# LorgeN/CART-SLAM

Measured on AMD Instinct MI355X. Metric: stereo-pairs/sec @1242x375xD=128; achieved HBM GB/s vs roofline, higher is better.
Workload: dtype u8

## Files before the change

### cart-slam_amd/cartslam/_lib.py

```python
import ctypes as C
import os

_HERE = os.path.dirname(os.path.abspath(__file__))
LIB_PATH = os.environ.get("CART_ENGINE_LIB") or os.path.join(os.path.dirname(_HERE), "build", "libcart_engine.so")


class EngineParams(C.Structure):
    _fields_ = [(n, C.c_int) for n in (
        "device_id", "width", "height", "min_disparity", "num_disparities", "paths", "p1", "p2",
        "uniqueness_ratio", "smoothing_radius", "smoothing_iterations", "max_inflight")]


class PlaneParams(C.Structure):
    _fields_ = [(n, C.c_int) for n in (
        "horizontal_min", "horizontal_max", "vertical_min", "vertical_max",
        "horizontal_center", "vertical_center")]

    def as_tuple(self):
        return tuple(getattr(self, n) for n, _ in self._fields_)


class LaunchPlan(C.Structure):
    _fields_ = [("frames_per_launch", C.c_int), ("plan", C.c_int), ("slabs_written", C.c_int)]


PLAN_AUTO, PLAN_SLABS, PLAN_FUSED_UP, PLAN_BAND_UP = -1, 0, 1, 2
OPT_PLAN, OPT_PLAN_MIN_FRAMES, OPT_CHUNK_FRAMES = 0, 1, 2
OPT_BAND_ROWS, OPT_BAND_PROBE = 6, 7
OPT_FLOW_GATHER = 8
OPT_SPEC_S8_ZERO_INVALID, OPT_SPEC_S7_REPLICATE_BORDER, OPT_SPEC_S5_TOP2 = 3, 4, 5


class FlowParams(C.Structure):
    _fields_ = [(n, C.c_int) for n in ("levels", "radius", "refine_radius", "block", "median")]


FLOW_MAX_LEVELS = 6


class PlacementReport(C.Structure):
    _fields_ = [("ms_first", C.c_float), ("ms_kept", C.c_float), ("ms_fastest_seen", C.c_float), ("ms_slowest_seen", C.c_float),
                ("seconds", C.c_float), ("units", C.c_int), ("candidates", C.c_int), ("mode", C.c_int), ("stop_reason", C.c_int)]


PRED_PLANEFIT, PRED_PLANECLUSTER = 0, 1
PLANEFIT_MAX_PLANES = 100
PLANEFIT_THRESHOLD = 0.01


ORB_DEFAULT_FEATURES, ORB_MAX_FEATURES, ORB_LEVELS, ORB_DESCRIPTOR_BYTES = 5000, 65536, 8, 32

# ... 356 lines not shown
```

### cart-slam_amd/cartslam/engine.py

```python
import collections
import ctypes as C

import numpy as np

from . import _lib
from ._lib import DenseEgoParams, ModelTrackColorParams, ModelTrackParams, EgoCamera, EgoParams, EngineParams, FusionParams, LocalBAParams, MatchParams, MotionParams, ObjectParams, PlaceParams, PlaneMapParams, PlaneParams, PoseGraphParams, SuperpixelParams, VoxelMapParams

INVALID = -32768


class EngineError(RuntimeError):
    pass


def _stream_ptr():
    import torch
    return C.c_void_p(torch.cuda.current_stream().cuda_stream)


def _geom(t, inner):
    if not t.is_cuda:
        raise EngineError("tensor must live on the GPU")
    batched = t.dim() == inner + 2
    if t.dim() not in (inner + 1, inner + 2):
# ... 82 lines not shown
    def __del__(self):
        try:
            self.close()
        except Exception:
            pass

    def _check(self, rc, what):
        if rc != 0:
            raise EngineError(f"{what}: " + self._lib.cart_last_error(self._h).decode())

    def set_plan(self, plan, min_frames=1):
        code = {"auto": _lib.PLAN_AUTO, "slabs": _lib.PLAN_SLABS, "fused_up": _lib.PLAN_FUSED_UP, "band_up": _lib.PLAN_BAND_UP}[plan]
        self._check(self._lib.cart_engine_set_option(self._h, _lib.OPT_PLAN, code), "cart_engine_set_option")
        self._check(self._lib.cart_engine_set_option(self._h, _lib.OPT_PLAN_MIN_FRAMES, int(min_frames)), "cart_engine_set_option")

    def set_spec_variants(self, s8_zero_invalid=False, s7_replicate_border=False, s5_top2=False):
        self._check(self._lib.cart_engine_set_option(self._h, _lib.OPT_SPEC_S5_TOP2, 1 if s5_top2 else 0), "cart_engine_set_option")
        self._check(self._lib.cart_engine_set_option(self._h, _lib.OPT_SPEC_S8_ZERO_INVALID, 1 if s8_zero_invalid else 0), "cart_engine_set_option")
        self._check(self._lib.cart_engine_set_option(self._h, _lib.OPT_SPEC_S7_REPLICATE_BORDER, 1 if s7_replicate_border else 0), "cart_engine_set_option")

    def set_band_rows(self, k, probe=False):
        self._check(self._lib.cart_engine_set_option(self._h, _lib.OPT_BAND_ROWS, int(k)), "cart_engine_set_option")
        self._check(self._lib.cart_engine_set_option(self._h, _lib.OPT_BAND_PROBE, 1 if probe else 0), "cart_engine_set_option")

    def set_chunk_frames(self, n):
        self._check(self._lib.cart_engine_set_option(self._h, _lib.OPT_CHUNK_FRAMES, int(n)), "cart_engine_set_option")

    def describe_plan(self, n_frames):
        lp = _lib.LaunchPlan()
        self._check(self._lib.cart_engine_describe_plan(self._h, int(n_frames), C.byref(lp)), "cart_engine_describe_plan")
        return {"frames_per_launch": lp.frames_per_launch, "plan": {0: "slabs", 1: "fused_up", 2: "band_up"}[lp.plan],
                "slabs_written": lp.slabs_written}

    def copy_narrow(self, dst, src, workgroups=0):
        nbytes = src.numel() * src.element_size()
        if dst.numel() * dst.element_size() != nbytes or not dst.is_contiguous() or not src.is_contiguous():
            raise EngineError("copy_narrow needs two contiguous tensors of the same byte size")
        if not (dst.is_cuda or dst.is_pinned()) or not (src.is_cuda or src.is_pinned()):
            raise EngineError("copy_narrow needs device tensors or pinned host tensors")
        self._check(self._lib.cart_copy_narrow(self._h, C.c_void_p(dst.data_ptr()), C.c_void_p(src.data_ptr()), nbytes, int(workgroups),
                                               _stream_ptr()), "cart_copy_narrow")
        return dst

    def tune_placement(self, n_frames, max_tries=8, max_extra_bytes=0, report=False):
        r = _lib.PlacementReport()
        cap = C.c_size_t(-1).value if max_extra_bytes is None else int(max_extra_bytes)
# ... 1512 lines not shown
```

### cart-slam_amd/csrc/cart_engine.hip

```cpp
#include <chrono>
#include <cstdio>

#include "engine_host.h"

using namespace cart_amd;

namespace cart_amd {

thread_local std::string g_last_error;
thread_local int g_last_slot = 0;

int fail(const std::string &msg) {
    g_last_error = msg;
    return -1;
}

int SlotLease::begin(cart_engine *e, int n, hipStream_t stream) {
    if (n <= 0 || n > (int)e->slots.size()) return fail("n_frames must be in [1, max_inflight]");
    std::unique_lock<std::mutex> lk(e->mu);
    int s0 = -1;
    for (;;) {
        const int total = (int)e->slots.size();
        int oldest = -1;
        unsigned long long oldest_seq = ~0ull;
// ... 79 lines not shown
    int blk = 0, nd = 0;
    const int lpb = agg_lines_per_block(g.D);
    for (int i = 0; i < g.P; ++i) {
        if (!((mask >> i) & 1u)) continue;
        DirDesc &d = a.dirs[nd++];
        d.dx = order8[i].dx; d.dy = order8[i].dy; d.path = order8[i].path;
        if (d.dy == 0) { d.nlines = g.h; d.jmin = 0; }
        else if (d.dx == 0) { d.nlines = g.w; d.jmin = 0; }
        else { d.nlines = g.w + g.h - 1; d.jmin = d.dx > 0 ? -(g.h - 1) : 0; }
        d.blk0 = blk;
        blk += (d.nlines + lpb - 1) / lpb;
    }
    a.ndirs = nd;
    a.blocks_per_frame = blk;
    a.cen_l = e->cen_l; a.cen_r = e->cen_r; a.slabs = SlabTable{};
}

struct Options {
    int plan, plan_min_frames, chunk_frames;
    bool timing;
    int spec;
    int band_rows;
    bool band_probe;
};
Options snapshot_options(const cart_engine *e) {
    return Options{e->opt_plan, e->opt_plan_min_frames, e->chunk_frames, e->timing, e->opt_spec, e->opt_band_rows, e->opt_band_probe != 0};
}

int plan_for(const cart_engine *e, const Options &o, int n) {
    if (o.spec & 4) return CART_PLAN_SLABS;
    const bool band_ok = wta_band_supported(e->g, o.band_rows, o.band_probe);
    if (o.plan == CART_PLAN_AUTO) {
        if (band_ok && !o.band_probe && n >= e->auto_band_min_frames) return CART_PLAN_BAND_UP;
        return n >= e->auto_fused_min_frames ? CART_PLAN_FUSED_UP : CART_PLAN_SLABS;
    }
    if (n < o.plan_min_frames) return CART_PLAN_SLABS;
    if (o.plan == CART_PLAN_BAND_UP && !band_ok) return CART_PLAN_SLABS;
    return o.plan;
}

int validate(const cart_engine_params *p) {
    if (!p) return fail("params is NULL");
    if (p->width < 16 || p->height < 8 || p->width > 16384 || p->height > 16384) return fail("unsupported image size");
    const bool post_only = p->num_disparities == 0 && p->paths == 0;
    if (!post_only && !(p->num_disparities == 64 || p->num_disparities == 128 || p->num_disparities == 256))
        return fail("num_disparities must be 64, 128 or 256");
    if (!post_only && !(p->paths == 4 || p->paths == 8)) return fail("paths must be 4 or 8");
    if (p->min_disparity < 0 || p->min_disparity > 64) return fail("min_disparity must be in [0, 64]");
    if (p->p1 < 0 || p->p2 < p->p1 || p->p2 + 31 > 255) return fail("need 0 <= p1 <= p2 and 31 + p2 <= 255");
// ... 54 lines not shown
    SlabTable t{};
    if (s0 < 0 || n < 1 || n > kMaxLaunchFrames || s0 + n > sp.slots || sp.group_slots < 1) return t;
    for (int f = 0; f < n; ++f) {
        const int s = s0 + f, gi = s / sp.group_slots;
        uint8_t *b = subst && (*subst)[gi] ? (*subst)[gi] : sp.base[gi];
        t.frame[f] = b + (size_t)(s % sp.group_slots) * sp.slot_bytes;
    }
    return t;
}

template <typename F>
void launch_agg_wta(cart_engine *e, const Options &opt, const SlabTable &slabs, size_t s0, int n, hipStream_t st, F between) {
    const Geometry &g = e->g;
    uint32_t *cl = e->cen_l + s0 * g.census_elems, *cr = e->cen_r + s0 * g.census_elems;
    uint16_t *wl = e->wta_l + s0 * g.npx;
    uint32_t *rpk = e->right_pk + s0 * g.npx;
    const int plan = plan_for(e, opt, n);
    const bool fused = plan == CART_PLAN_FUSED_UP && e->rv_partial, band = plan == CART_PLAN_BAND_UP;
    AggArgs a = fused ? e->agg_fused : e->agg;
    a.cen_l = cl; a.cen_r = cr; a.slabs = slabs;
    a.ckpt_rows = band && !opt.band_probe ? opt.band_rows : 0;
    launch_aggregate(a, n, st);
    between();
    if (band) launch_wta_band(cl, cr, slabs, wl, rpk, g, e->uniq_thr, n, opt.band_rows, opt.band_probe, st);
    else if (fused) launch_wta_fused(cl, cr, slabs, wl, rpk, e->rv_partial + s0 * wta_fused_partial_elems(g), g, e->uniq_thr, n, st);
    else launch_wta(slabs, wl, rpk, g, e->uniq_thr, n, st, (opt.spec & 4) != 0);
}

}

extern "C" {

void cart_engine_default_params(cart_engine_params *p) {
    if (!p) return;
    std::memset(p, 0, sizeof(*p));
    p->device_id = 0;
    p->min_disparity = 4;
    p->num_disparities = 256;
    p->paths = 4;
    p->p1 = 10; p->p2 = 120;
    p->uniqueness_ratio = 12;
    p->smoothing_radius = -1;
    p->smoothing_iterations = 5;
    p->max_inflight = 12;
}

int cart_engine_create(const cart_engine_params *params, cart_engine **out) {
// ... 88 lines not shown
    if (!e) return fail("engine is NULL");
    std::lock_guard<std::mutex> lk(e->mu);
    switch (option) {
        case CART_OPT_PLAN:
            if (value < CART_PLAN_AUTO || value > CART_PLAN_BAND_UP) return fail("unknown plan");
            e->opt_plan = value;
            return 0;
        case CART_OPT_PLAN_MIN_FRAMES:
            if (value < 1) return fail("min frames must be >= 1");
            e->opt_plan_min_frames = value;
            return 0;
        case CART_OPT_CHUNK_FRAMES:
            if (value < 1 || value > kMaxLaunchFrames) return fail("chunk frames must be in [1, 64]");
            e->chunk_frames = value;
            return 0;
        case CART_OPT_BAND_ROWS:
            if (value != 1 && value != 4 && value != 8 && value != 16) return fail("band rows must be 4, 8 or 16 (1 with the probe)");
            e->opt_band_rows = value;
            return 0;
        case CART_OPT_BAND_PROBE:
            if (value != 0 && value != 1) return fail("the band probe is 0 or 1");
            e->opt_band_probe = value;
            return 0;
        case CART_OPT_FLOW_GATHER:
            if (value != 0 && value != 1) return fail("the flow gather option is 0 or 1");
            e->opt_flow_gather = value;
            return 0;
        case CART_OPT_SPEC_S8_ZERO_INVALID:
        case CART_OPT_SPEC_S7_REPLICATE_BORDER:
        case CART_OPT_SPEC_S5_TOP2: {
            if (value != 0 && value != 1) return fail("spec variants are 0 or 1");
            const int bit = option == CART_OPT_SPEC_S8_ZERO_INVALID ? 1 : option == CART_OPT_SPEC_S7_REPLICATE_BORDER ? 2 : 4;
            e->opt_spec = value ? (e->opt_spec | bit) : (e->opt_spec & ~bit);
            return 0;
        }
        default: return fail("unknown option");
    }
}

int cart_engine_get_option(cart_engine *e, int option, int *value) {
    if (!e || !value) return fail("bad arguments");
    std::lock_guard<std::mutex> lk(e->mu);
    switch (option) {
        case CART_OPT_PLAN: *value = e->opt_plan; return 0;
        case CART_OPT_PLAN_MIN_FRAMES: *value = e->opt_plan_min_frames; return 0;
        case CART_OPT_CHUNK_FRAMES: *value = e->chunk_frames; return 0;
        case CART_OPT_BAND_ROWS: *value = e->opt_band_rows; return 0;
        case CART_OPT_BAND_PROBE: *value = e->opt_band_probe; return 0;
        case CART_OPT_FLOW_GATHER: *value = e->opt_flow_gather; return 0;
        case CART_OPT_SPEC_S8_ZERO_INVALID: *value = (e->opt_spec & 1) ? 1 : 0; return 0;
        case CART_OPT_SPEC_S7_REPLICATE_BORDER: *value = (e->opt_spec & 2) ? 1 : 0; return 0;
        case CART_OPT_SPEC_S5_TOP2: *value = (e->opt_spec & 4) ? 1 : 0; return 0;
        default: return fail("unknown option");
    }
}

int cart_engine_describe_plan(cart_engine *e, int n_frames, cart_launch_plan *out) {
    if (!e || !out) return fail("bad arguments");
    if (e->post_only) return fail("this engine was created without SGM workspaces (num_disparities = 0)");
    if (n_frames < 1) return fail("n_frames must be positive");
    std::lock_guard<std::mutex> lk(e->mu);
    const Options o = snapshot_options(e);
    out->frames_per_launch = std::min(n_frames, o.chunk_frames);
    out->plan = plan_for(e, o, out->frames_per_launch);
    out->slabs_written = out->plan == CART_PLAN_FUSED_UP || (out->plan == CART_PLAN_BAND_UP && !o.band_probe) ? e->g.P - 1 : e->g.P;
    return 0;
}

namespace {
float probe_placement(cart_engine *e, const Options &opt, const SlabTable &slabs, size_t s0, int n, hipEvent_t ev0, hipEvent_t ev1) {
    const Geometry &g = e->g;
// ... 394 lines not shown
```

### cart-slam_amd/csrc/engine_host.h

```cpp
#pragma once

#include <algorithm>
#include <cmath>
#include <condition_variable>
#include <cstring>
#include <mutex>
#include <new>
#include <string>
#include <vector>

#include "engine_internal.h"

#pragma GCC visibility push(hidden)

namespace cart_amd {

extern thread_local std::string g_last_error;
extern thread_local int g_last_slot;

int fail(const std::string &msg);

int check_positive(const char *name, double v);
int check_camera(const cart_ego_camera *cam);
int check_pose(const char *name, const double *m);
// ... 13 lines not shown
};
int check_pitched(const Extent &x);
bool overlap(const Extent &a, const Extent &b);
int check_outputs_apart(const Extent *all, int first_output, int n);

#define HIP_TRY(expr)                                                                               \
    do {                                                                                            \
        hipError_t _e = (expr);                                                                     \
        if (_e != hipSuccess)                                                                       \
            return fail(std::string(#expr) + ": " + hipGetErrorString(_e) + " (" + __FILE__ + ":" + \
                        std::to_string(__LINE__) + ")");                                           \
    } while (0)

struct Slot {
    bool busy = false;
    hipEvent_t done = nullptr;
    int owner = -1;
    hipStream_t last_stream = nullptr;
    bool used = false;
    unsigned long long released_seq = 0;
};

constexpr int kBandRowsDefault = 8;
constexpr int kBandAutoMinFrames = 4;
constexpr int kMaxTimings = 8;
constexpr int kTimingRing = 256;

struct TimingRec {
    hipEvent_t ev[kMaxTimings + 1] = {};
    const char *names[kMaxTimings] = {};
    int n = 0;
};

struct SlabPool {
    std::vector<uint8_t *> base;
    int group_slots = 0;
    int slots = 0;
    size_t slot_bytes = 0;
    int groups() const { return (int)base.size(); }
    int slots_of(int gi) const { return std::min(group_slots, slots - gi * group_slots); }
    size_t bytes_of(int gi) const { return (size_t)slots_of(gi) * slot_bytes; }
    uint8_t *slot_ptr(int s) const { return base[s / group_slots] + (size_t)(s % group_slots) * slot_bytes; }
};

}

// ... 3 lines not shown
    float uniq;
    uint16_t *uniq_thr = nullptr;
    uint8_t *gray_l = nullptr, *gray_r = nullptr;
    uint32_t *cen_l = nullptr, *cen_r = nullptr;
    uint32_t *cen_l_alloc = nullptr, *cen_r_alloc = nullptr;
    size_t cen_slack = 0;
    uint16_t *wta_l = nullptr;
    uint32_t *right_pk = nullptr;
    int16_t *tmp_a = nullptr, *tmp_b = nullptr;
    int32_t *ccl_work = nullptr;
    uint32_t *rv_partial = nullptr;
    uint8_t *flow_ws = nullptr;
    uint8_t *flow_pyr_ws = nullptr;
    int32_t *ccl_stats_ws = nullptr;
    unsigned *sp_votes = nullptr;
    std::vector<void *> bufs;
    cart_amd::AggArgs agg;
    cart_amd::AggArgs agg_fused;
    cart_amd::SlabPool slab_pool;
    int auto_fused_min_frames = 1 << 30;
    int opt_plan = CART_PLAN_AUTO;
    int auto_band_min_frames = 1 << 30;
    int opt_band_rows = cart_amd::kBandRowsDefault, opt_band_probe = 0;
    int opt_plan_min_frames = 1;
    int opt_flow_gather = 0;
    int opt_spec = 0;
    std::mutex mu;
    std::condition_variable cv;
    std::vector<cart_amd::Slot> slots;
    unsigned long long release_counter = 0;
    int chunk_frames = cart_amd::kLaunchFrames;
    bool post_only = false;
    bool timing = false;
    int timing_every = 1;
    unsigned long long timing_calls = 0;
    std::vector<cart_amd::TimingRec> ring;
    size_t ring_calls = 0;
};

namespace cart_amd {

class SlotLease {
   public:
    SlotLease() = default;
    SlotLease(const SlotLease &) = delete;
    SlotLease &operator=(const SlotLease &) = delete;
// ... 83 lines not shown
```

### cart-slam_amd/csrc/engine_internal.h

```cpp
#pragma once

#include <hip/hip_runtime.h>
#include <stddef.h>
#include <stdint.h>

#include "cart_engine.h"

namespace cart_amd {

constexpr int kMaxPaths = 8;
constexpr int kWtaTileX = 64;
constexpr int kMaxBatchArgs = 128;
constexpr uint32_t kWtaInvalid = 0xFFFFu;
constexpr int kSlabChunkOrder[16] = {0, 8, 1, 9, 2, 10, 3, 11, 4, 12, 5, 13, 6, 14, 7, 15};

struct Geometry {
    int w, h, D, P;
    int min_disp, p1, p2;
    int cpitch;
    int cpadl;
    size_t npx;
    size_t census_elems;
    size_t slab_bytes;
};
// ... 34 lines not shown
    ImageBatch b{}; b.ptr = ptr; b.step = step; b.frame_stride = frame_stride; return b;
}

struct OutBatch {
    int16_t *ptr;
    size_t step, frame_stride;
    int16_t *frames[kLaunchFrames];
    int scattered;
};
inline OutBatch strided_out(int16_t *ptr, size_t step, size_t frame_stride) {
    OutBatch b{}; b.ptr = ptr; b.step = step; b.frame_stride = frame_stride; return b;
}

void launch_census(const ImageBatch &left, const ImageBatch &right, int channels, int n_frames,
                   uint8_t *gray_l, uint8_t *gray_r, uint32_t *cen_l, uint32_t *cen_r, uint32_t *right_pk,
                   const Geometry &g, hipStream_t s);
int agg_lines_per_block(int D);
int agg_residency_cap(int ndirs, int D, int n_frames, bool hsplit = false);
bool agg_hsplit(const Geometry &g, int ndirs, int n_frames);
void launch_aggregate(const AggArgs &a, int n_frames, hipStream_t s);
void launch_wta(const SlabTable &slabs, uint16_t *wta_l, uint32_t *right_pk, const Geometry &g, const uint16_t *thr,
                int n_frames, hipStream_t s, bool top2 = false);
constexpr int kUpPath = 1;
size_t wta_fused_partial_elems(const Geometry &g);
void launch_wta_fused(const uint32_t *cen_l, const uint32_t *cen_r, const SlabTable &slabs, uint16_t *wta_l, uint32_t *right_pk,
                      uint32_t *partial, const Geometry &g, const uint16_t *thr, int n_frames, hipStream_t s);
bool wta_band_supported(const Geometry &g, int K, bool probe);
void launch_wta_band(const uint32_t *cen_l, const uint32_t *cen_r, const SlabTable &slabs, uint16_t *wta_l, uint32_t *right_pk,
                     const Geometry &g, const uint16_t *thr, int n_frames, int K, bool probe, hipStream_t s);
void launch_uniq_table(float u, uint16_t *out_dev, hipStream_t s);
void uniq_table_host(float u, uint16_t *out);
void launch_post(const uint16_t *wta_l, const uint32_t *right_pk, const uint8_t *gray_l, const OutBatch &out, const Geometry &g, int n_frames, hipStream_t s,
                 int spec = 0);
bool post_interp_fusable(int radius, int min_disp16, int max_disp);
void launch_post_interp(const uint16_t *wta_l, const uint32_t *right_pk, const uint8_t *gray_l, const OutBatch &out, const Geometry &g, int n_frames,
                        hipStream_t s, int spec, int min_disp16, int max_disp);

void launch_interpolate(const int16_t *src, size_t src_step, size_t src_fs, const OutBatch &dst, int w, int h, int radius,
                        int min_disp16, int max_disp, int n_frames, hipStream_t s);
void launch_dir_derivative(const int16_t *disp, size_t step, size_t fs, int16_t *out, size_t ostep, size_t ofs,
                           int32_t *hist512, int w, int h, int n_frames, hipStream_t s);
struct FrameTable { const void *p[kLaunchFrames]; int scattered; };
void launch_plane_derivative(const int16_t *disp, size_t step, size_t fs, int16_t *out, size_t ostep, size_t ofs,
                             int32_t *hist256, size_t hist_fs, int w, int h, int n_frames, hipStream_t s,
                             const FrameTable *disp_table = nullptr, const FrameTable *out_table = nullptr);
struct ClassifyParams { cart_plane_params p[kMaxBatchArgs]; };
void launch_classify(const int16_t *deriv, size_t step, size_t fs, const ClassifyParams &params, int per_frame,
                     uint8_t *planes, size_t pstep, size_t pfs, int w, int h, int n_frames, hipStream_t s,
                     const FrameTable *deriv_table = nullptr, const FrameTable *planes_table = nullptr);
void launch_ccl(const uint8_t *planes, size_t pstep, size_t pfs, int32_t *work, int32_t *ids, size_t istep, size_t ifs,
                int32_t *ncomp, int w, int h, int n_frames, hipStream_t s, int32_t *stat = nullptr, int32_t *seg = nullptr,
                cart_component *table = nullptr, int max_components = 0);
// ... 598 lines not shown
```

### cart-slam_amd/csrc/sgm_aggregate.hip

```cpp
#include <algorithm>

#include "sgm_device.h"

namespace cart_amd {


typedef uint32_t u32x4_g4 __attribute__((ext_vector_type(4), aligned(4)));
__device__ __forceinline__ void ld_u32x16(const uint32_t *ubase, unsigned &byte_off, uint32_t (&r)[16]) {
    const CART_GLOBAL char *b = (const CART_GLOBAL char *)sgpr(ubase) + pin_v(byte_off);
#pragma unroll
    for (int i = 0; i < 4; ++i) {
        const u32x4_g4 v = *(const CART_GLOBAL u32x4_g4 *)(b + 16 * i);
        r[4 * i + 0] = v.x; r[4 * i + 1] = v.y; r[4 * i + 2] = v.z; r[4 * i + 3] = v.w;
    }
}

__device__ __forceinline__ void load_census(const uint32_t *pl, unsigned &off_l, const uint32_t *pr, unsigned &off_r, CensusRegs &c) {
    c.fl = ld_u32(pl, off_l);
    ld_u32x16(pr, off_r, c.r);
}

constexpr int HS_PF = 8;
template <int LPP, int DX>
__device__ __forceinline__ void hscan_sliding(uint32_t (&st)[8], uint32_t &mm, const uint32_t *&pl, unsigned &lo_l, const uint32_t *&pr,
// ... 9 lines not shown
    }
    auto group = [&]() {
#pragma unroll
        for (int j = 0; j < 16; ++j) {
            constexpr int M = 15;
            const int slot = j % HS_PF;
#pragma unroll
            for (int k = 0; k < 16; ++k) xr[k] = ffl[slot] ^ win[(DX > 0 ? k + j : k - j + 16) & M];
            win[(DX > 0 ? j : 15 - j) & M] = fnw[slot];
            __builtin_amdgcn_sched_barrier(0);
            ffl[slot] = ld_u32(pl + (j + HS_PF) * DX, lo_l);
            fnw[slot] = ld_u32(pr + (j + HS_PF + 1) * DX, lo_n);
            __builtin_amdgcn_sched_barrier(0);
            agg_step<LPP>(st, mm, xr, sel_lo, sel_hi, p1p1, p2p2, sgpr(po + j * ostride) + pin_v(lo_o));
            __builtin_amdgcn_sched_barrier(0);
        }
        pl += 16 * DX; pr += 16 * DX; po += 16 * ostride;
    };
    group();
    for (int gi = 1; gi < groups; ++gi) group();
}

constexpr int kHsCostDwords = 2 * 2 * 64 * 4;

template <int LPP>
__device__ __forceinline__ v4u agg_step_c(uint32_t (&a)[8], uint32_t &mm, const uint32_t (&c)[8], uint32_t sel_lo, uint32_t sel_hi,
                                          uint32_t p1p1, uint32_t p2p2) {
    const uint32_t mp2 = mm + p2p2;
    const uint32_t lo0 = perm(a[7], dpp_mov<DPP_ROW_SHR1>(a[7]), sel_lo);
    const uint32_t hi7 = perm(dpp_mov<DPP_ROW_SHL1>(a[0]), a[0], sel_hi);
    uint32_t n[8];
#pragma unroll
    for (int i = 0; i < 8; ++i) {
        const uint32_t lo = i == 0 ? lo0 : a[i - 1];
        const uint32_t hi = i == 7 ? hi7 : a[i + 1];
        uint32_t t = pk_min(lo, hi) + p1p1;
        t = pk_min3(t, a[i], mp2);
        n[i] = (t - mm) + c[i];
    }
    const v4u q = {perm(n[1], n[0], 0x06040200u), perm(n[3], n[2], 0x06040200u), perm(n[5], n[4], 0x06040200u), perm(n[7], n[6], 0x06040200u)};
    uint32_t x = pk_min(pk_min3(n[0], n[1], n[2]), pk_min3(n[3], n[4], pk_min3(n[5], n[6], n[7])));
    x = pk_min(x, __builtin_amdgcn_alignbit(x, x, 16));
    mm = group_allmin<LPP>(x);
#pragma unroll
    for (int i = 0; i < 8; ++i) a[i] = n[i];
    return q;
}

template <int LPP, int DX>
__device__ __forceinline__ void hsplit_producer(const uint32_t *pl, unsigned lo_l, const uint32_t *pr, unsigned lo_r, int w, uint32_t *cost, int lane) {
    auto emit = [&](int parity, const uint32_t (&c)[8]) {
        v4u *dst = reinterpret_cast<v4u *>(cost) + parity * 128 + lane;
        dst[0] = v4u{c[0], c[1], c[2], c[3]};
        dst[64] = v4u{c[4], c[5], c[6], c[7]};
        lds_barrier();
    };
    const int groups = w / 16;
    if (groups > 0) {
        uint32_t win[16], ffl[HS_PF], fnw[HS_PF];
        ld_u32x16(pr, lo_r, win);
        unsigned lo_n = lo_r + (DX > 0 ? 15u * 4u : 0u);
#pragma unroll
        for (int q = 0; q < HS_PF; ++q) {
            ffl[q] = ld_u32(pl + q * DX, lo_l);
            fnw[q] = ld_u32(pr + (q + 1) * DX, lo_n);
        }
        auto group = [&]() {
#pragma unroll
            for (int j = 0; j < 16; ++j) {
                const int slot = j % HS_PF;
// ... 346 lines not shown
```

### cart-slam_amd/csrc/sgm_device.h

```cpp
#pragma once

#include <type_traits>

#include "engine_internal.h"

namespace cart_amd {

typedef uint16_t u16x2 __attribute__((ext_vector_type(2)));
typedef uint32_t v4u __attribute__((ext_vector_type(4)));

__device__ __forceinline__ uint32_t pk_min(uint32_t a, uint32_t b) {
    return __builtin_bit_cast(uint32_t, __builtin_elementwise_min(__builtin_bit_cast(u16x2, a), __builtin_bit_cast(u16x2, b)));
}
__device__ __forceinline__ uint32_t pk_min3(uint32_t a, uint32_t b, uint32_t c) {
#if defined(__gfx950__)
    uint32_t r;
    asm("v_pk_minimum3_f16 %0, %1, %2, %3" : "=v"(r) : "v"(a), "v"(b), "v"(c));
    return r;
#else
    return pk_min(pk_min(a, b), c);
#endif
}
__device__ __forceinline__ void keep_f16_denormals() { __builtin_amdgcn_s_setreg(1 | (6 << 6) | (1 << 11), 3); }
__device__ __forceinline__ uint32_t pk_add(uint32_t a, uint32_t b) {
// ... 84 lines not shown
        uint32_t t = pk_min(lo, hi) + p1p1;
        t = pk_min3(t, a[i], mp2);
        uint32_t u = t - mm;
        asm volatile("" : "+v"(u));
        uint32_t lo_sum = (uint32_t)__builtin_popcount(xr[15 - i]) + u;
        asm volatile("" : "+v"(lo_sum));
        n[i] = ((uint32_t)__builtin_popcount(xr[7 - i]) << 16) + lo_sum;
    }
    if constexpr (STORE) {
        uint4 o;
        o.x = perm(n[1], n[0], 0x06040200u); o.y = perm(n[3], n[2], 0x06040200u);
        o.z = perm(n[5], n[4], 0x06040200u); o.w = perm(n[7], n[6], 0x06040200u);
        const v4u q = {o.x, o.y, o.z, o.w};
        if (store_row) __builtin_nontemporal_store(q, (CART_GLOBAL v4u *)po);
    } else {
        (void)po; (void)store_row;
    }
    mm = path_min<LPP>(n);
#pragma unroll
    for (int i = 0; i < 8; ++i) a[i] = n[i];
}

template <int LPP>
struct Win {
    static constexpr int P = 64 / LPP;
    static constexpr int D = 16 * LPP;
    static constexpr int RL = 16 + P - 1;
    static constexpr int RS = LPP == 4 ? 40 : LPP == 8 ? 36 : 34;
    static constexpr int NE = LPP * RL;
    static constexpr int NLD = (NE + 63) / 64;
    static constexpr int BUF = LPP * RS;
    static_assert(RS >= RL && RS % 32 == (P / 2) % 32, "region stride");
};

template <int LPP>
struct WinLane {
    unsigned goff[Win<LPP>::NLD];
    int lslot[Win<LPP>::NLD];
    int rbase;
    __device__ __forceinline__ void init(int lane) {
        using WN = Win<LPP>;
#pragma unroll
        for (int i = 0; i < WN::NLD; ++i) {
            const int e = min(64 * i + lane, WN::NE - 1);
            const int g = e / WN::RL, o = e - g * WN::RL;
            goff[i] = (unsigned)(WN::D - 16 - 16 * g + o) * 4u;
// ... 29 lines not shown
```

### cart-slam_amd/csrc/sgm_wta.hip

```cpp
#include <cstdlib>
#include <type_traits>

#include "sgm_device.h"

namespace cart_amd {

__host__ __device__ constexpr int rv_slot(int i) { return i + (i >> 4); }
__host__ __device__ constexpr int rv_size(int n) { return ((n + (n >> 4) + 1) + 3) & ~3; }
__host__ __device__ constexpr int rv_row_slots(int cols, int D, bool padded) { return ((padded ? rv_size(cols + D - 1) : cols + D) + 7) & ~7; }
__host__ __device__ constexpr uint32_t rv_key16(uint32_t key32, int cols) {
    return ((((key32 >> 16) << (cols == 32 ? 5 : 4)) | (key32 & (uint32_t)(cols - 1))) & 0xffffu);
}
__host__ __device__ constexpr uint32_t rv_key32(uint32_t key16, int e, int cols, int D) {
    const int sh = cols == 32 ? 5 : 4, base = D - 1 - e;
    return ((key16 >> sh) << 16) | (uint32_t)(base + (((int)(key16 & (uint32_t)(cols - 1)) - base) & (cols - 1)));
}

__device__ __forceinline__ uint32_t pk_sub_sat(uint32_t a, uint32_t b) {
    return __builtin_bit_cast(uint32_t, __builtin_elementwise_sub_sat(__builtin_bit_cast(u16x2, a), __builtin_bit_cast(u16x2, b)));
}

__host__ __device__ __forceinline__ uint32_t uniq_threshold(uint32_t bc, float u) {
    if (bc == 0) return 0;
    if (!(u > 0.f)) return 4095u;
// ... 136 lines not shown
        p1p1 = (uint32_t)g.p1 * 0x10001u; p2p2 = (uint32_t)g.p2 * 0x10001u;
        sel_lo = gl == 0 ? 0x05040d0du : 0x05040302u;
        sel_hi = gl == LPP - 1 ? 0x0d0d0302u : 0x05040302u;
        wl.init(lane);
        const ptrdiff_t cen0 = (ptrdiff_t)frame * (ptrdiff_t)g.census_elems + g.cpadl + xw0;
        pw0 = cen_r + uniform(cen0 - g.min_disp - (D - 1));
        pl0 = cen_l + uniform(cen0);
        lo_l = (unsigned)pg * 4u;
        const int xbase = min(xw0, g.w - 1), xc = min(x, g.w - 1);
        ps0 = slabs + uniform((ptrdiff_t)xbase * D);
        lo_s = (unsigned)((xc - xbase) * D + d0);
        cpitch = g.cpitch; row_bytes = (ptrdiff_t)g.w * D; slab_bytes = (ptrdiff_t)g.slab_bytes;
    }
    __device__ __forceinline__ void load_census_row(int y, uint32_t (&win)[WN::NLD], uint32_t &fl) {
        const uint32_t *pw = pw0 + (ptrdiff_t)y * cpitch;
#pragma unroll
        for (int i = 0; i < WN::NLD; ++i) win[i] = ld_u32(pw, wl.goff[i]);
        fl = ld_u32(pl0 + (ptrdiff_t)y * cpitch, lo_l);
    }
    __device__ __forceinline__ v4u load_slab(int y, int path) {
        const uint8_t *ps = ps0 + (ptrdiff_t)y * row_bytes + (ptrdiff_t)path * slab_bytes;
        return __builtin_nontemporal_load((const CART_GLOBAL v4u *)((const CART_GLOBAL char *)sgpr(ps) + pin_v(lo_s)));
    }
    template <bool SKIP_UP, int NS>
    __device__ __forceinline__ void load_slab_row(int y, uint32_t (&sv)[NS][4]) {
#pragma unroll
        for (int p = 0; p < (SKIP_UP ? NS + 1 : NS); ++p) {
            if (SKIP_UP && p == kUpPath) continue;
            const int k = SKIP_UP && p > kUpPath ? p - 1 : p;
            const v4u v = load_slab(y, p);
            sv[k][0] = v.x; sv[k][1] = v.y; sv[k][2] = v.z; sv[k][3] = v.w;
        }
    }
};

template <int LPP, bool TOP2 = false>
__global__ __launch_bounds__(256) void wta_kernel(WtaArgs a) {
    extern __shared__ __attribute__((aligned(16))) uint16_t s_lds[];
    constexpr int D = LPP * 16;
    constexpr int DP = D + 8;
    constexpr int PPP = 256 / LPP;
    constexpr int NPASS = kWtaTileX / PPP;
    uint16_t *wta_l = a.wta_l;
    uint32_t *right_pk = a.right_pk;
    const Geometry &g = a.g;
    const int x0 = blockIdx.x * kWtaTileX, y = blockIdx.y, frame = blockIdx.z;
    const uint8_t *slabs = a.slabs.frame[frame];
    const int grp = threadIdx.x / LPP, gl = threadIdx.x % LPP, d0 = gl * 16;
    __shared__ uint32_t s_rv[kWtaTileX + D];
    for (int i = threadIdx.x; i < kWtaTileX + D; i += 256) s_rv[i] = 0xffffffffu;
    __syncthreads();

// ... 85 lines not shown
}

void launch_wta(const SlabTable &slabs, uint16_t *wta_l, uint32_t *right_pk, const Geometry &g, const uint16_t *thr,
                int n_frames, hipStream_t s, bool top2) {
    dim3 grid((g.w + kWtaTileX - 1) / kWtaTileX, g.h, n_frames), block(256);
    const size_t lds = (size_t)kWtaTileX * (g.D + 8) * sizeof(uint16_t);
    WtaArgs a{slabs, wta_l, right_pk, g, thr, g.P, {0, 1, 2, 3, 4, 5, 6, 7}};
    with_lpp(g.D, [&](auto lpp) {
        constexpr int LPP = decltype(lpp)::value;
        if (top2) hipLaunchKernelGGL((wta_kernel<LPP, true>), grid, block, lds, s, a);
        else hipLaunchKernelGGL((wta_kernel<LPP>), grid, block, lds, s, a);
    });
}

struct BandArgs {
    const uint32_t *cen_l, *cen_r;
    SlabTable slabs;
    uint16_t *wta_l;
    uint32_t *right_pk;
    Geometry g;
    const uint16_t *thr;
};

template <int LPP, int K, bool RECOMP = true>
__global__ __launch_bounds__(64 * LPP, 4) void wta_band_kernel(BandArgs a) {
    using WN = Win<LPP>;
    constexpr int D = WN::D, P = WN::P, NT = 64 * LPP, NP = kMaxPaths, NS = RECOMP ? NP - 1 : NP;
    constexpr int DP = D + 8;
    constexpr int NRV = kWtaTileX + D;
    static_assert(P * LPP == 64 && NT / LPP == kWtaTileX, "one pixel of the tile per lane group");
    __shared__ __attribute__((aligned(16))) uint16_t s_sum[kWtaTileX * DP];
    __shared__ uint32_t s_rv[2][NRV];
    __shared__ uint32_t s_win[RECOMP ? LPP : 1][WN::BUF];
    __shared__ uint16_t s_thr[2048];
    const Geometry &g = a.g;
    keep_f16_denormals();
    const int x0 = blockIdx.x * kWtaTileX, frame = blockIdx.z;
    const int y0 = (int)blockIdx.y * K, y1 = min(g.h, y0 + K);

    for (int i = threadIdx.x; i < 2 * NRV; i += NT) (&s_rv[0][0])[i] = 0xffffffffu;
    for (int i = threadIdx.x; i < 2048; i += NT) s_thr[i] = a.thr[i];

    UpSweep<LPP> sw;
    sw.init(g, a.cen_l, a.cen_r, a.slabs.frame[frame], frame, x0);
    const int gl = sw.gl, d0 = sw.d0, xl = sw.xl, x = sw.x;
    const bool valid = sw.valid;
    uint32_t *wbuf = &s_win[RECOMP ? sw.wid : 0][0];
    uint32_t cw[WN::NLD], cfl, sv[NS][4];

    uint32_t st[8], mm = 0;
#pragma unroll
    for (int i = 0; i < 8; ++i) st[i] = 0;
    if constexpr (RECOMP) sw.load_census_row(y1 - 1, cw, cfl);
    if (RECOMP && y1 < g.h) {
        const v4u v = sw.load_slab(y1, kUpPath);
#pragma unroll
        for (int q = 0; q < 4; ++q) {
            st[2 * q] = perm(0u, v[q], 0x0c010c00u);
            st[2 * q + 1] = perm(0u, v[q], 0x0c030c02u);
        }
        mm = path_min<LPP>(st);
    }
    sw.template load_slab_row<RECOMP>(y1 - 1, sv);
    lds_barrier();

    auto row = [&](int y, auto last_c) {
        constexpr bool LAST = decltype(last_c)::value;
        uint32_t *rvb = &s_rv[y & 1][0];
        uint32_t sm[8];
        if constexpr (RECOMP) {
#pragma unroll
            for (int i = 0; i < WN::NLD; ++i) wbuf[sw.wl.lslot[i]] = cw[i];
            CensusRegs c;
            c.fl = cfl;
            win_read<LPP>(wbuf, sw.wl.rbase, c.r);
            uint32_t xr[16];
            agg_xor(c, xr);
            if constexpr (!LAST) sw.load_census_row(y - 1, cw, cfl);
            agg_step<LPP, false>(st, mm, xr, sw.sel_lo, sw.sel_hi, sw.p1p1, sw.p2p2, nullptr);
            sum_from_state(sm, st);
        } else {
#pragma unroll
            for (int k = 0; k < 8; ++k) sm[k] = 0;
        }
#pragma unroll
        for (int k = 0; k < NS; ++k) sum_add_slab(sm, sv[k]);
        if constexpr (!LAST) sw.template load_slab_row<RECOMP>(y - 1, sv);
        v4u *dst = reinterpret_cast<v4u *>(s_sum + xl * DP + d0);
        dst[0] = v4u{sm[0], sm[1], sm[2], sm[3]};
        dst[1] = v4u{sm[4], sm[5], sm[6], sm[7]};
        if (valid) rv_scatter(rvb + (xl + D - 1 - d0), sm, d0);
        uint32_t pk, T, tot;
        wta_best_and_sum<LPP>(sm, d0, s_thr, pk, T, tot);
        if (gl == 0 && valid) {
            const WtaPick w = wta_decide<D>(pk, T, tot, s_sum + xl * DP);
            a.wta_l[(size_t)frame * g.npx + (size_t)y * g.w + x] = (uint16_t)wta_subpixel<D>(w);
        }
        lds_barrier();
        for (int pi = threadIdx.x; pi < kWtaTileX + D - 1; pi += NT) {
            const int p = x0 - (D - 1) + pi;
            const uint32_t best = rvb[pi];
            rvb[pi] = 0xffffffffu;
            if (p >= 0 && p < g.w && best != 0xffffffffu) atomicMin(&a.right_pk[(size_t)frame * g.npx + (size_t)y * g.w + p], best);
        }
    };
    for (int y = y1 - 1; y > y0; --y) row(y, std::false_type{});
    row(y0, std::true_type{});
}

bool wta_band_supported(const Geometry &g, int K, bool probe) { return g.D == 128 && g.P == kMaxPaths && (K == 4 || K == 8 || K == 16 || (probe && K == 1)); }

void launch_wta_band(const uint32_t *cen_l, const uint32_t *cen_r, const SlabTable &slabs, uint16_t *wta_l, uint32_t *right_pk,
                     const Geometry &g, const uint16_t *thr, int n_frames, int K, bool probe, hipStream_t s) {
    dim3 grid((g.w + kWtaTileX - 1) / kWtaTileX, (g.h + K - 1) / K, n_frames), block(64 * (g.D / 16));
    BandArgs a{cen_l, cen_r, slabs, wta_l, right_pk, g, thr};
    if (probe) {
        switch (K) {
            case 1: hipLaunchKernelGGL((wta_band_kernel<8, 1, false>), grid, block, 0, s, a); break;
            case 4: hipLaunchKernelGGL((wta_band_kernel<8, 4, false>), grid, block, 0, s, a); break;
            case 8: hipLaunchKernelGGL((wta_band_kernel<8, 8, false>), grid, block, 0, s, a); break;
            default: hipLaunchKernelGGL((wta_band_kernel<8, 16, false>), grid, block, 0, s, a); break;
        }
        return;
    }
    switch (K) {
        case 4: hipLaunchKernelGGL((wta_band_kernel<8, 4>), grid, block, 0, s, a); break;
        case 8: hipLaunchKernelGGL((wta_band_kernel<8, 8>), grid, block, 0, s, a); break;
        default: hipLaunchKernelGGL((wta_band_kernel<8, 16>), grid, block, 0, s, a); break;
    }
}

constexpr int fused_waves(int lpp) { return lpp >= 16 ? 4 : 2; }
constexpr int kFusedRB = 16;
inline int fused_waves_for(const Geometry &g) { return g.D >= 256 && g.w >= 1600 ? 2 * fused_waves(16) : fused_waves(g.D / 16); }


struct FusedArgs {
    const uint32_t *cen_l, *cen_r;
    SlabTable slabs;
    uint16_t *wta_l;
    uint32_t *partial;
    Geometry g;
    const uint16_t *thr;
    int xcd_frames;
// ... 263 lines not shown
```

### include/cart_engine.h

```cpp
#ifndef CART_ENGINE_H
#define CART_ENGINE_H

#include <stddef.h>
#include <stdint.h>

#ifdef __cplusplus
extern "C" {
#endif

#define CART_DISPARITY_INVALID (-32768)

enum { CART_PLANE_HORIZONTAL = 0, CART_PLANE_VERTICAL = 1, CART_PLANE_UNKNOWN = 2 };

typedef struct cart_engine cart_engine;

typedef struct {
    int device_id;
    int width, height;
    int min_disparity;
    int num_disparities;
    int paths;
    int p1, p2;
    int uniqueness_ratio;
    int smoothing_radius;
// ... 2 lines not shown
} cart_engine_params;

typedef struct {
    int horizontal_min, horizontal_max;
    int vertical_min, vertical_max;
    int horizontal_center, vertical_center;
} cart_plane_params;

void cart_engine_default_params(cart_engine_params *p);

int cart_engine_create(const cart_engine_params *params, cart_engine **out);
void cart_engine_destroy(cart_engine *engine);

enum { CART_PLAN_AUTO = -1, CART_PLAN_SLABS = 0, CART_PLAN_FUSED_UP = 1, CART_PLAN_BAND_UP = 2 };
enum {
    CART_OPT_PLAN = 0,
    CART_OPT_PLAN_MIN_FRAMES = 1,
    CART_OPT_CHUNK_FRAMES = 2,
    CART_OPT_SPEC_S8_ZERO_INVALID = 3,
    CART_OPT_SPEC_S7_REPLICATE_BORDER = 4,
    CART_OPT_SPEC_S5_TOP2 = 5,
    CART_OPT_BAND_ROWS = 6,
    CART_OPT_BAND_PROBE = 7,
    CART_OPT_FLOW_GATHER = 8
};
int cart_engine_set_option(cart_engine *engine, int option, int value);
int cart_engine_get_option(cart_engine *engine, int option, int *value);
typedef struct {
    int frames_per_launch;
    int plan;
    int slabs_written;
} cart_launch_plan;
int cart_engine_describe_plan(cart_engine *engine, int n_frames, cart_launch_plan *out);

enum { CART_PLACE_MODE_UNKNOWN = 0, CART_PLACE_MODE_FAST = 1, CART_PLACE_MODE_MIXED = 2, CART_PLACE_MODE_UNIFORM = 3 };
enum { CART_PLACE_STOP_NOTHING_TO_DO = 0, CART_PLACE_STOP_FAST_FOUND = 1, CART_PLACE_STOP_UNIFORM = 2, CART_PLACE_STOP_TRIES = 3,
       CART_PLACE_STOP_TIME = 4, CART_PLACE_STOP_MEMORY = 5 };
typedef struct {
    float ms_first, ms_kept;
    float ms_fastest_seen, ms_slowest_seen;
    float seconds;
    int units, candidates;
    int mode, stop_reason;
} cart_placement_report;
int cart_engine_tune_placement(cart_engine *engine, int n_frames, int max_tries, size_t max_extra_bytes, cart_placement_report *report);

const char *cart_last_error(const cart_engine *engine);
// ... 600 lines not shown
```

Measured before the change: 5965.

## Recompute the up-right diagonal path inside the band WTA kernel

The band WTA kernel can now recompute the up-right diagonal aggregation path in registers, alongside the already recomputed vertical up path, instead of loading that path's cost slab for every row. Neighbouring lanes exchange their diagonal state each row through a double-buffered shared-memory array, and the tile's left-edge column is read from the slab. The row is seeded from the slab at the band's bottom boundary. The aim is to cut the per-row HBM slab reads in the WTA pass, at the cost of more ALU work, extra LDS traffic and higher register pressure. A new option, on by default, selects the diagonal variant whenever the band plan runs.

```diff
diff --git a/cart-slam_amd/cartslam/_lib.py b/cart-slam_amd/cartslam/_lib.py
--- a/cart-slam_amd/cartslam/_lib.py
+++ b/cart-slam_amd/cartslam/_lib.py
@@ -27,6 +27,7 @@
 PLAN_AUTO, PLAN_SLABS, PLAN_FUSED_UP, PLAN_BAND_UP = -1, 0, 1, 2
 OPT_PLAN, OPT_PLAN_MIN_FRAMES, OPT_CHUNK_FRAMES = 0, 1, 2
 OPT_BAND_ROWS, OPT_BAND_PROBE = 6, 7
+OPT_BAND_DIAG = 9
 OPT_FLOW_GATHER = 8
 OPT_SPEC_S8_ZERO_INVALID, OPT_SPEC_S7_REPLICATE_BORDER, OPT_SPEC_S5_TOP2 = 3, 4, 5
 
diff --git a/cart-slam_amd/cartslam/engine.py b/cart-slam_amd/cartslam/engine.py
--- a/cart-slam_amd/cartslam/engine.py
+++ b/cart-slam_amd/cartslam/engine.py
@@ -128,6 +128,14 @@
     def set_band_rows(self, k, probe=False):
         self._check(self._lib.cart_engine_set_option(self._h, _lib.OPT_BAND_ROWS, int(k)), "cart_engine_set_option")
         self._check(self._lib.cart_engine_set_option(self._h, _lib.OPT_BAND_PROBE, 1 if probe else 0), "cart_engine_set_option")
+
+    def set_band_diag(self, on=True):
+        self._check(self._lib.cart_engine_set_option(self._h, _lib.OPT_BAND_DIAG, 1 if on else 0), "cart_engine_set_option")
+
+    def get_option(self, option):
+        v = C.c_int(0)
+        self._check(self._lib.cart_engine_get_option(self._h, int(option), C.byref(v)), "cart_engine_get_option")
+        return int(v.value)
 
     def set_chunk_frames(self, n):
         self._check(self._lib.cart_engine_set_option(self._h, _lib.OPT_CHUNK_FRAMES, int(n)), "cart_engine_set_option")
diff --git a/cart-slam_amd/csrc/cart_engine.hip b/cart-slam_amd/csrc/cart_engine.hip
--- a/cart-slam_amd/csrc/cart_engine.hip
+++ b/cart-slam_amd/csrc/cart_engine.hip
@@ -125,9 +125,10 @@
     int spec;
     int band_rows;
     bool band_probe;
+    bool band_diag;
 };
 Options snapshot_options(const cart_engine *e) {
-    return Options{e->opt_plan, e->opt_plan_min_frames, e->chunk_frames, e->timing, e->opt_spec, e->opt_band_rows, e->opt_band_probe != 0};
+    return Options{e->opt_plan, e->opt_plan_min_frames, e->chunk_frames, e->timing, e->opt_spec, e->opt_band_rows, e->opt_band_probe != 0, e->opt_band_diag != 0};
 }
 
 int plan_for(const cart_engine *e, const Options &o, int n) {
@@ -228,7 +229,7 @@
     a.ckpt_rows = band && !opt.band_probe ? opt.band_rows : 0;
     launch_aggregate(a, n, st);
     between();
-    if (band) launch_wta_band(cl, cr, slabs, wl, rpk, g, e->uniq_thr, n, opt.band_rows, opt.band_probe, st);
+    if (band) launch_wta_band(cl, cr, slabs, wl, rpk, g, e->uniq_thr, n, opt.band_rows, opt.band_probe, opt.band_diag, st);
     else if (fused) launch_wta_fused(cl, cr, slabs, wl, rpk, e->rv_partial + s0 * wta_fused_partial_elems(g), g, e->uniq_thr, n, st);
     else launch_wta(slabs, wl, rpk, g, e->uniq_thr, n, st, (opt.spec & 4) != 0);
 }
@@ -363,6 +364,10 @@
             if (value != 0 && value != 1) return fail("the band probe is 0 or 1");
             e->opt_band_probe = value;
             return 0;
+        case CART_OPT_BAND_DIAG:
+            if (value != 0 && value != 1) return fail("the band diagonal option is 0 or 1");
+            e->opt_band_diag = value;
+            return 0;
         case CART_OPT_FLOW_GATHER:
             if (value != 0 && value != 1) return fail("the flow gather option is 0 or 1");
             e->opt_flow_gather = value;
@@ -388,6 +393,7 @@
         case CART_OPT_CHUNK_FRAMES: *value = e->chunk_frames; return 0;
         case CART_OPT_BAND_ROWS: *value = e->opt_band_rows; return 0;
         case CART_OPT_BAND_PROBE: *value = e->opt_band_probe; return 0;
+        case CART_OPT_BAND_DIAG: *value = e->opt_band_diag; return 0;
         case CART_OPT_FLOW_GATHER: *value = e->opt_flow_gather; return 0;
         case CART_OPT_SPEC_S8_ZERO_INVALID: *value = (e->opt_spec & 1) ? 1 : 0; return 0;
         case CART_OPT_SPEC_S7_REPLICATE_BORDER: *value = (e->opt_spec & 2) ? 1 : 0; return 0;
diff --git a/cart-slam_amd/csrc/engine_host.h b/cart-slam_amd/csrc/engine_host.h
--- a/cart-slam_amd/csrc/engine_host.h
+++ b/cart-slam_amd/csrc/engine_host.h
@@ -59,6 +59,7 @@
 };
 
 constexpr int kBandRowsDefault = 8;
+constexpr int kBandDiagDefault = 1;
 constexpr int kBandAutoMinFrames = 4;
 constexpr int kMaxTimings = 8;
 constexpr int kTimingRing = 256;
@@ -108,6 +109,7 @@
     int opt_plan = CART_PLAN_AUTO;
     int auto_band_min_frames = 1 << 30;
     int opt_band_rows = cart_amd::kBandRowsDefault, opt_band_probe = 0;
+    int opt_band_diag = cart_amd::kBandDiagDefault;
     int opt_plan_min_frames = 1;
     int opt_flow_gather = 0;
     int opt_spec = 0;
diff --git a/cart-slam_amd/csrc/engine_internal.h b/cart-slam_amd/csrc/engine_internal.h
--- a/cart-slam_amd/csrc/engine_internal.h
+++ b/cart-slam_amd/csrc/engine_internal.h
@@ -80,12 +80,13 @@
 void launch_wta(const SlabTable &slabs, uint16_t *wta_l, uint32_t *right_pk, const Geometry &g, const uint16_t *thr,
                 int n_frames, hipStream_t s, bool top2 = false);
 constexpr int kUpPath = 1;
+constexpr int kUpRightPath = 7;
 size_t wta_fused_partial_elems(const Geometry &g);
 void launch_wta_fused(const uint32_t *cen_l, const uint32_t *cen_r, const SlabTable &slabs, uint16_t *wta_l, uint32_t *right_pk,
                       uint32_t *partial, const Geometry &g, const uint16_t *thr, int n_frames, hipStream_t s);
 bool wta_band_supported(const Geometry &g, int K, bool probe);
 void launch_wta_band(const uint32_t *cen_l, const uint32_t *cen_r, const SlabTable &slabs, uint16_t *wta_l, uint32_t *right_pk,
-                     const Geometry &g, const uint16_t *thr, int n_frames, int K, bool probe, hipStream_t s);
+                     const Geometry &g, const uint16_t *thr, int n_frames, int K, bool probe, bool diag, hipStream_t s);
 void launch_uniq_table(float u, uint16_t *out_dev, hipStream_t s);
 void uniq_table_host(float u, uint16_t *out);
 void launch_post(const uint16_t *wta_l, const uint32_t *right_pk, const uint8_t *gray_l, const OutBatch &out, const Geometry &g, int n_frames, hipStream_t s,
diff --git a/cart-slam_amd/csrc/sgm_aggregate.hip b/cart-slam_amd/csrc/sgm_aggregate.hip
--- a/cart-slam_amd/csrc/sgm_aggregate.hip
+++ b/cart-slam_amd/csrc/sgm_aggregate.hip
@@ -55,30 +55,6 @@
 }
 
 constexpr int kHsCostDwords = 2 * 2 * 64 * 4;
-
-template <int LPP>
-__device__ __forceinline__ v4u agg_step_c(uint32_t (&a)[8], uint32_t &mm, const uint32_t (&c)[8], uint32_t sel_lo, uint32_t sel_hi,
-                                          uint32_t p1p1, uint32_t p2p2) {
-    const uint32_t mp2 = mm + p2p2;
-    const uint32_t lo0 = perm(a[7], dpp_mov<DPP_ROW_SHR1>(a[7]), sel_lo);
-    const uint32_t hi7 = perm(dpp_mov<DPP_ROW_SHL1>(a[0]), a[0], sel_hi);
-    uint32_t n[8];
-#pragma unroll
-    for (int i = 0; i < 8; ++i) {
-        const uint32_t lo = i == 0 ? lo0 : a[i - 1];
-        const uint32_t hi = i == 7 ? hi7 : a[i + 1];
-        uint32_t t = pk_min(lo, hi) + p1p1;
-        t = pk_min3(t, a[i], mp2);
-        n[i] = (t - mm) + c[i];
-    }
-    const v4u q = {perm(n[1], n[0], 0x06040200u), perm(n[3], n[2], 0x06040200u), perm(n[5], n[4], 0x06040200u), perm(n[7], n[6], 0x06040200u)};
-    uint32_t x = pk_min(pk_min3(n[0], n[1], n[2]), pk_min3(n[3], n[4], pk_min3(n[5], n[6], n[7])));
-    x = pk_min(x, __builtin_amdgcn_alignbit(x, x, 16));
-    mm = group_allmin<LPP>(x);
-#pragma unroll
-    for (int i = 0; i < 8; ++i) a[i] = n[i];
-    return q;
-}
 
 template <int LPP, int DX>
 __device__ __forceinline__ void hsplit_producer(const uint32_t *pl, unsigned lo_l, const uint32_t *pr, unsigned lo_r, int w, uint32_t *cost, int lane) {
diff --git a/cart-slam_amd/csrc/sgm_device.h b/cart-slam_amd/csrc/sgm_device.h
--- a/cart-slam_amd/csrc/sgm_device.h
+++ b/cart-slam_amd/csrc/sgm_device.h
@@ -130,6 +130,30 @@
 }
 
 template <int LPP>
+__device__ __forceinline__ v4u agg_step_c(uint32_t (&a)[8], uint32_t &mm, const uint32_t (&c)[8], uint32_t sel_lo, uint32_t sel_hi,
+                                          uint32_t p1p1, uint32_t p2p2) {
+    const uint32_t mp2 = mm + p2p2;
+    const uint32_t lo0 = perm(a[7], dpp_mov<DPP_ROW_SHR1>(a[7]), sel_lo);
+    const uint32_t hi7 = perm(dpp_mov<DPP_ROW_SHL1>(a[0]), a[0], sel_hi);
+    uint32_t n[8];
+#pragma unroll
+    for (int i = 0; i < 8; ++i) {
+        const uint32_t lo = i == 0 ? lo0 : a[i - 1];
+        const uint32_t hi = i == 7 ? hi7 : a[i + 1];
+        uint32_t t = pk_min(lo, hi) + p1p1;
+        t = pk_min3(t, a[i], mp2);
+        n[i] = (t - mm) + c[i];
+    }
+    const v4u q = {perm(n[1], n[0], 0x06040200u), perm(n[3], n[2], 0x06040200u), perm(n[5], n[4], 0x06040200u), perm(n[7], n[6], 0x06040200u)};
+    uint32_t x = pk_min(pk_min3(n[0], n[1], n[2]), pk_min3(n[3], n[4], pk_min3(n[5], n[6], n[7])));
+    x = pk_min(x, __builtin_amdgcn_alignbit(x, x, 16));
+    mm = group_allmin<LPP>(x);
+#pragma unroll
+    for (int i = 0; i < 8; ++i) a[i] = n[i];
+    return q;
+}
+
+template <int LPP>
 struct Win {
     static constexpr int P = 64 / LPP;
     static constexpr int D = 16 * LPP;
diff --git a/cart-slam_amd/csrc/sgm_wta.hip b/cart-slam_amd/csrc/sgm_wta.hip
--- a/cart-slam_amd/csrc/sgm_wta.hip
+++ b/cart-slam_amd/csrc/sgm_wta.hip
@@ -182,12 +182,13 @@
         const uint8_t *ps = ps0 + (ptrdiff_t)y * row_bytes + (ptrdiff_t)path * slab_bytes;
         return __builtin_nontemporal_load((const CART_GLOBAL v4u *)((const CART_GLOBAL char *)sgpr(ps) + pin_v(lo_s)));
     }
-    template <bool SKIP_UP, int NS>
+    template <bool SKIP_UP, bool SKIP_UR = false, int NS>
     __device__ __forceinline__ void load_slab_row(int y, uint32_t (&sv)[NS][4]) {
 #pragma unroll
-        for (int p = 0; p < (SKIP_UP ? NS + 1 : NS); ++p) {
+        for (int p = 0; p < NS + (SKIP_UP ? 1 : 0) + (SKIP_UR ? 1 : 0); ++p) {
             if (SKIP_UP && p == kUpPath) continue;
-            const int k = SKIP_UP && p > kUpPath ? p - 1 : p;
+            if (SKIP_UR && p == kUpRightPath) continue;
+            const int k = p - (SKIP_UP && p > kUpPath ? 1 : 0) - (SKIP_UR && p > kUpRightPath ? 1 : 0);
             const v4u v = load_slab(y, p);
             sv[k][0] = v.x; sv[k][1] = v.y; sv[k][2] = v.z; sv[k][3] = v.w;
         }
@@ -319,10 +320,11 @@
     const uint16_t *thr;
 };
 
-template <int LPP, int K, bool RECOMP = true>
+template <int LPP, int K, bool RECOMP = true, bool DIAG = false>
 __global__ __launch_bounds__(64 * LPP, 4) void wta_band_kernel(BandArgs a) {
     using WN = Win<LPP>;
-    constexpr int D = WN::D, P = WN::P, NT = 64 * LPP, NP = kMaxPaths, NS = RECOMP ? NP - 1 : NP;
+    static_assert(RECOMP || !DIAG, "the diagonal shares the matching costs of the \"up\" recompute");
+    constexpr int D = WN::D, P = WN::P, NT = 64 * LPP, NP = kMaxPaths, NS = RECOMP ? (DIAG ? NP - 2 : NP - 1) : NP;
     constexpr int DP = D + 8;
     constexpr int NRV = kWtaTileX + D;
     static_assert(P * LPP == 64 && NT / LPP == kWtaTileX, "one pixel of the tile per lane group");
@@ -330,6 +332,7 @@
     __shared__ uint32_t s_rv[2][NRV];
     __shared__ uint32_t s_win[RECOMP ? LPP : 1][WN::BUF];
     __shared__ uint16_t s_thr[2048];
+    __shared__ v4u s_dg[DIAG ? 2 : 1][DIAG ? NT : 1];
     const Geometry &g = a.g;
     keep_f16_denormals();
     const int x0 = blockIdx.x * kWtaTileX, frame = blockIdx.z;
@@ -344,6 +347,16 @@
     const bool valid = sw.valid;
     uint32_t *wbuf = &s_win[RECOMP ? sw.wid : 0][0];
     uint32_t cw[WN::NLD], cfl, sv[NS][4];
+    const uint8_t *pc0 = nullptr;
+    unsigned lo_c = (unsigned)d0;
+    v4u cv = {0u, 0u, 0u, 0u};
+    bool colz = true;
+    const int dg_wr = (int)threadIdx.x, dg_rd = xl == 0 ? dg_wr : dg_wr - LPP;
+    if constexpr (DIAG) pc0 = a.slabs.frame[frame] + uniform((ptrdiff_t)kUpRightPath * (ptrdiff_t)g.slab_bytes + (ptrdiff_t)max(x0 - 1, 0) * D);
+    auto load_col = [&](int yy) {
+        const uint8_t *pc = pc0 + (ptrdiff_t)yy * sw.row_bytes;
+        return __builtin_nontemporal_load((const CART_GLOBAL v4u *)((const CART_GLOBAL char *)sgpr(pc) + pin_v(lo_c)));
+    };
 
     uint32_t st[8], mm = 0;
 #pragma unroll
@@ -358,7 +371,16 @@
         }
         mm = path_min<LPP>(st);
     }
-    sw.template load_slab_row<RECOMP>(y1 - 1, sv);
+    if constexpr (DIAG) {
+        v4u seed = {0u, 0u, 0u, 0u};
+        if (y1 < g.h) seed = sw.load_slab(y1, kUpRightPath);
+        cv = load_col(min(y1, g.h - 1));
+        colz = x0 == 0 || y1 >= g.h;
+        sw.template load_slab_row<RECOMP, DIAG>(y1 - 1, sv);
+        s_dg[y1 & 1][dg_wr] = seed;
+    } else {
+        sw.template load_slab_row<RECOMP>(y1 - 1, sv);
+    }
     lds_barrier();
 
     auto row = [&](int y, auto last_c) {
@@ -374,15 +396,39 @@
             uint32_t xr[16];
             agg_xor(c, xr);
             if constexpr (!LAST) sw.load_census_row(y - 1, cw, cfl);
-            agg_step<LPP, false>(st, mm, xr, sw.sel_lo, sw.sel_hi, sw.p1p1, sw.p2p2, nullptr);
-            sum_from_state(sm, st);
+            if constexpr (DIAG) {
+                uint32_t mc[8];
+#pragma unroll
+                for (int i = 0; i < 8; ++i) mc[i] = ((uint32_t)__builtin_popcount(xr[7 - i]) << 16) + (uint32_t)__builtin_popcount(xr[15 - i]);
+                (void)agg_step_c<LPP>(st, mm, mc, sw.sel_lo, sw.sel_hi, sw.p1p1, sw.p2p2);
+                sum_from_state(sm, st);
+                const v4u nb = s_dg[(y + 1) & 1][dg_rd];
+                const bool edge = xl == 0;
+                uint32_t pv[4], ds[8];
+#pragma unroll
+                for (int q = 0; q < 4; ++q) {
+                    pv[q] = edge ? (colz ? 0u : cv[q]) : nb[q];
+                    ds[2 * q] = perm(0u, pv[q], 0x0c010c00u);
+                    ds[2 * q + 1] = perm(0u, pv[q], 0x0c030c02u);
+                }
+                uint32_t dm = path_min<LPP>(ds);
+                const v4u dq = agg_step_c<LPP>(ds, dm, mc, sw.sel_lo, sw.sel_hi, sw.p1p1, sw.p2p2);
+                s_dg[y & 1][dg_wr] = dq;
+                sum_add_slab(sm, dq);
+            } else {
+                agg_step<LPP, false>(st, mm, xr, sw.sel_lo, sw.sel_hi, sw.p1p1, sw.p2p2, nullptr);
+                sum_from_state(sm, st);
+            }
         } else {
 #pragma unroll
             for (int k = 0; k < 8; ++k) sm[k] = 0;
         }
 #pragma unroll
         for (int k = 0; k < NS; ++k) sum_add_slab(sm, sv[k]);
-        if constexpr (!LAST) sw.template load_slab_row<RECOMP>(y - 1, sv);
+        if constexpr (!LAST) {
+            if constexpr (DIAG) cv = load_col(y);
+            sw.template load_slab_row<RECOMP, DIAG>(y - 1, sv);
+        }
         v4u *dst = reinterpret_cast<v4u *>(s_sum + xl * DP + d0);
         dst[0] = v4u{sm[0], sm[1], sm[2], sm[3]};
         dst[1] = v4u{sm[4], sm[5], sm[6], sm[7]};
@@ -401,14 +447,17 @@
             if (p >= 0 && p < g.w && best != 0xffffffffu) atomicMin(&a.right_pk[(size_t)frame * g.npx + (size_t)y * g.w + p], best);
         }
     };
-    for (int y = y1 - 1; y > y0; --y) row(y, std::false_type{});
+    for (int y = y1 - 1; y > y0; --y) {
+        row(y, std::false_type{});
+        if constexpr (DIAG) colz = x0 == 0;
+    }
     row(y0, std::true_type{});
 }
 
 bool wta_band_supported(const Geometry &g, int K, bool probe) { return g.D == 128 && g.P == kMaxPaths && (K == 4 || K == 8 || K == 16 || (probe && K == 1)); }
 
 void launch_wta_band(const uint32_t *cen_l, const uint32_t *cen_r, const SlabTable &slabs, uint16_t *wta_l, uint32_t *right_pk,
-                     const Geometry &g, const uint16_t *thr, int n_frames, int K, bool probe, hipStream_t s) {
+                     const Geometry &g, const uint16_t *thr, int n_frames, int K, bool probe, bool diag, hipStream_t s) {
     dim3 grid((g.w + kWtaTileX - 1) / kWtaTileX, (g.h + K - 1) / K, n_frames), block(64 * (g.D / 16));
     BandArgs a{cen_l, cen_r, slabs, wta_l, right_pk, g, thr};
     if (probe) {
@@ -417,6 +466,14 @@
             case 4: hipLaunchKernelGGL((wta_band_kernel<8, 4, false>), grid, block, 0, s, a); break;
             case 8: hipLaunchKernelGGL((wta_band_kernel<8, 8, false>), grid, block, 0, s, a); break;
             default: hipLaunchKernelGGL((wta_band_kernel<8, 16, false>), grid, block, 0, s, a); break;
+        }
+        return;
+    }
+    if (diag) {
+        switch (K) {
+            case 4: hipLaunchKernelGGL((wta_band_kernel<8, 4, true, true>), grid, block, 0, s, a); break;
+            case 8: hipLaunchKernelGGL((wta_band_kernel<8, 8, true, true>), grid, block, 0, s, a); break;
+            default: hipLaunchKernelGGL((wta_band_kernel<8, 16, true, true>), grid, block, 0, s, a); break;
         }
         return;
     }
diff --git a/include/cart_engine.h b/include/cart_engine.h
--- a/include/cart_engine.h
+++ b/include/cart_engine.h
@@ -48,7 +48,8 @@
     CART_OPT_SPEC_S5_TOP2 = 5,
     CART_OPT_BAND_ROWS = 6,
     CART_OPT_BAND_PROBE = 7,
-    CART_OPT_FLOW_GATHER = 8
+    CART_OPT_FLOW_GATHER = 8,
+    CART_OPT_BAND_DIAG = 9
 };
 int cart_engine_set_option(cart_engine *engine, int option, int value);
 int cart_engine_get_option(cart_engine *engine, int option, int *value);
```

Measured after the change: 6169, median of 6. +3.4%, better.
